# djene-mengistu/UAPS

Hardware: NVIDIA B200
Metric: fused_pl_kl_loss_pixels_per_s (higher is better)
Workload: dtype f32

## Files before the change

uaps_b200/csrc/common.cuh:

```cuda
#pragma once
#include <cuda_runtime.h>
#include <stdint.h>
#include <cstdlib>
#include "uaps_b200.h"

#define UAPS_API extern "C" __attribute__((visibility("default")))

#define UAPS_LAUNCH_CHECK()                                   \
    do {                                                      \
        cudaError_t e__ = cudaGetLastError();                 \
        if (e__ != cudaSuccess) return (int)e__;              \
    } while (0)

namespace uaps {

constexpr int kWarp = 32;

struct DeviceInfo { int sm_count; int cc_major; int cc_minor; };
inline const DeviceInfo& device_info() {
    static const DeviceInfo info = [] {
        DeviceInfo d{148, 10, 0};
        int dev = 0;
        if (cudaGetDevice(&dev) == cudaSuccess) {
            cudaDeviceGetAttribute(&d.sm_count, cudaDevAttrMultiProcessorCount, dev);
            cudaDeviceGetAttribute(&d.cc_major, cudaDevAttrComputeCapabilityMajor, dev);
            cudaDeviceGetAttribute(&d.cc_minor, cudaDevAttrComputeCapabilityMinor, dev);
        }
        return d;
    }();
    return info;
}

template <typename T> __host__ __device__ constexpr T ceil_div(T a, T b) { return (a + b - 1) / b; }

__device__ __forceinline__ void grid_dep_wait() { asm volatile("griddepcontrol.wait;" ::: "memory"); }
__device__ __forceinline__ void grid_dep_launch() { asm volatile("griddepcontrol.launch_dependents;" ::: "memory"); }
inline bool pdl_all_enabled() {
    static const bool on = [] { const char* e = getenv("UAPS_PDL"); return e != nullptr && atoi(e) != 0; }();
    return on;
}
template <typename... KArgs, typename... Args>
inline cudaError_t launch_k(void (*kern)(KArgs...), dim3 grid, dim3 block, size_t smem, cudaStream_t st, bool cooperative,
                            Args... args) {
    cudaLaunchConfig_t cfg{};
    cfg.gridDim = grid; cfg.blockDim = block; cfg.dynamicSmemBytes = smem; cfg.stream = st;
    cudaLaunchAttribute attr[2];
    int n = 0;
    if (pdl_all_enabled()) {
        attr[n].id = cudaLaunchAttributeProgrammaticStreamSerialization;
        attr[n].val.programmaticStreamSerializationAllowed = 1;
        ++n;
    }
    if (cooperative) {
        attr[n].id = cudaLaunchAttributeCooperative;
        attr[n].val.cooperative = 1;
        ++n;
    }
    cfg.attrs = attr; cfg.numAttrs = n;
    return cudaLaunchKernelEx(&cfg, kern, KArgs(args)...);
}
#define UAPS_LAUNCH(kern, grid, block, smem, stream, ...)                                          \
    do {                                                                                           \
        cudaError_t le__ = ::uaps::launch_k(kern, grid, block, smem, stream, false, __VA_ARGS__);  \
        if (le__ != cudaSuccess) return (int)le__;                                                 \
    } while (0)

inline bool aligned_to(const void* p, size_t a) { return (reinterpret_cast<uintptr_t>(p) % a) == 0; }

template <int VEC> struct VecF;
template <> struct VecF<4> { using type = float4; };
template <> struct VecF<2> { using type = float2; };
template <> struct VecF<1> { using type = float;  };

template <int VEC>
__device__ __forceinline__ void load_vec(const float* __restrict__ p, float (&out)[VEC]) {
    using V = typename VecF<VEC>::type;
    V v = __ldg(reinterpret_cast<const V*>(p));
    const float* f = reinterpret_cast<const float*>(&v);
#pragma unroll
    for (int i = 0; i < VEC; ++i) out[i] = f[i];
}
template <int VEC>
__device__ __forceinline__ void store_vec(float* __restrict__ p, const float (&in)[VEC]) {
    using V = typename VecF<VEC>::type;
    V v;
    float* f = reinterpret_cast<float*>(&v);
#pragma unroll
    for (int i = 0; i < VEC; ++i) f[i] = in[i];
    *reinterpret_cast<V*>(p) = v;
}

__device__ __forceinline__ float warp_sum(float v) {
#pragma unroll
    for (int o = 16; o > 0; o >>= 1) v += __shfl_xor_sync(0xffffffffu, v, o);
    return v;
}
__device__ __forceinline__ double warp_sum(double v) {
#pragma unroll
    for (int o = 16; o > 0; o >>= 1) v += __shfl_xor_sync(0xffffffffu, v, o);
    return v;
}
__device__ __forceinline__ float warp_max(float v) {
#pragma unroll
    for (int o = 16; o > 0; o >>= 1) v = fmaxf(v, __shfl_xor_sync(0xffffffffu, v, o));
    return v;
}

__host__ __device__ __forceinline__ uint32_t enc_ordered(float f) {
#ifdef __CUDA_ARCH__
// ... 35 lines not shown
```

uaps_b200/csrc/fused_loss.cu:

```cuda
#define UAPS_LOSS_ENTRY
#include <cstdlib>
#include <cstring>
#include "fused_loss_impl.cuh"

namespace uaps {
namespace loss {
#define UAPS_DECL_K(KK)                                                                                       \
    extern template int launch_loss_k<KK>(int, int, bool, bool, const LossArgs&, float*, const float*,       \
                                          const float*, int*, cudaStream_t);
UAPS_DECL_K(1) UAPS_DECL_K(2) UAPS_DECL_K(3) UAPS_DECL_K(4) UAPS_DECL_K(5) UAPS_DECL_K(6)
#undef UAPS_DECL_K
}

namespace {
using namespace loss;

int check_common(const float* const* z, int K, int B, int C, int64_t HW, const float* mix_w,
                 const int64_t* labels, const float* wcw_dev) {
    if (z == nullptr || B <= 0 || HW <= 0) return UAPS_EINVAL;
    if (K < 1 || K > KMAX || C < 2 || C > CMAX) return UAPS_ERANGE;
    if (labels == nullptr && mix_w == nullptr && wcw_dev == nullptr) return UAPS_EINVAL;
    if ((double)B * (double)HW >= 2147483648.0) return UAPS_ERANGE;
    for (int k = 0; k < K; ++k) {
        if (z[k] == nullptr) return UAPS_EINVAL;
        if (!aligned_to(z[k], 4)) return UAPS_EALIGN;
    }
    if (labels != nullptr && !aligned_to(labels, 8)) return UAPS_EALIGN;
    return UAPS_OK;
}

int pick_vec(const float* const* z, float* const* o, int K, int64_t HW) {
    int vec = (HW % 4 == 0) ? 4 : (HW % 2 == 0 ? 2 : 1);
    for (int k = 0; k < K; ++k) {
        while (vec > 1 && !aligned_to(z[k], 4 * vec)) vec >>= 1;
        if (o != nullptr && o[k] != nullptr)
            while (vec > 1 && !aligned_to(o[k], 4 * vec)) vec >>= 1;
    }
    return vec;
}


int pick_impl(int avail_vec, int flags, bool pass2, int kc) {
    static const int forced = [] { const char* e = getenv("UAPS_LOSS_IMPL"); return e ? atoi(e) : -1; }();
    static const int forced_p1 = [] { const char* e = getenv("UAPS_LOSS_P1_IMPL"); return e ? atoi(e) : -1; }();
    if (flags & UAPS_LOSS_EXACT) return IMPL_EXACT;
    if (avail_vec < 2) return IMPL_SCALAR;
    if (!pass2 && forced_p1 >= 0 && forced_p1 != IMPL_EXACT && forced_p1 <= IMPL_VEC4 && (forced_p1 != IMPL_VEC4 || avail_vec >= 4) &&
        (forced_p1 != IMPL_VEC4_PF || avail_vec >= 4))
        return forced_p1;
    if (forced >= 0 && forced <= IMPL_SCALAR) return forced;
    if (avail_vec < 4) return IMPL_VEC2_PF;
    static const int p2_vec4_max_kc = [] { const char* e = getenv("UAPS_LOSS_P2_VEC4_MAXKC"); return e ? atoi(e) : 12; }();
    if (pass2) return kc <= p2_vec4_max_kc ? IMPL_VEC4_PF : IMPL_VEC2_PF;
    return IMPL_VEC4_PF;
}

int dispatch_k(int K, int C, int impl, bool sup, bool pass2, const LossArgs& a, float* partials, const float* sc,
               const float* go, int* nblocks, cudaStream_t st) {
    switch (K) {
        case 1: return launch_loss_k<1>(C, impl, sup, pass2, a, partials, sc, go, nblocks, st);
        case 2: return launch_loss_k<2>(C, impl, sup, pass2, a, partials, sc, go, nblocks, st);
        case 3: return launch_loss_k<3>(C, impl, sup, pass2, a, partials, sc, go, nblocks, st);
        case 4: return launch_loss_k<4>(C, impl, sup, pass2, a, partials, sc, go, nblocks, st);
        case 5: return launch_loss_k<5>(C, impl, sup, pass2, a, partials, sc, go, nblocks, st);
        case 6: return launch_loss_k<6>(C, impl, sup, pass2, a, partials, sc, go, nblocks, st);
    }
    return UAPS_ERANGE;
}


constexpr int XCHG_WMAX = UAPS_XCHG_MAX_RANKS;
constexpr int XCHG_SLOT = 128;
constexpr size_t XCHG_WORDS = (size_t)2 * XCHG_WMAX * 2 * XCHG_SLOT;
constexpr size_t XCHG_STATUS_OFF = XCHG_WORDS * sizeof(unsigned long long);
constexpr size_t XCHG_BYTES = XCHG_STATUS_OFF + 128;
static_assert(sums_count(KMAX, CMAX) <= XCHG_SLOT, "slot too small");

struct ExchangeArgs {
    char* box[XCHG_WMAX];
    int rank, world;
    unsigned epoch;
    const unsigned* epoch_dev;
    unsigned long long timeout_ns;
};

__device__ __forceinline__ void st_word_sys(unsigned long long* p, unsigned data, unsigned flag) {
    asm volatile("st.volatile.global.v2.u32 [%0], {%1, %2};" ::"l"(p), "r"(data), "r"(flag) : "memory");
}
__device__ __forceinline__ void ld_word_sys(const unsigned long long* p, unsigned& data, unsigned& flag) {
    asm volatile("ld.volatile.global.v2.u32 {%0, %1}, [%2];" : "=r"(data), "=r"(flag) : "l"(p) : "memory");
}
__device__ __forceinline__ unsigned long long global_timer_ns() {
    unsigned long long t;
    asm volatile("mov.u64 %0, %%globaltimer;" : "=l"(t));
    return t;
}

__global__ void __launch_bounds__(1024) loss_fold_exchange_finalize_kernel(const float* __restrict__ partials, int S, unsigned nblocks,
                                                                            double* __restrict__ sums, const ExchangeArgs x, int K,
                                                                            int C, double N, float cw1, float cw2, int supervised,
                                                                            float* __restrict__ sc, int nsc,
                                                                            const float* __restrict__ wcw_dev) {
    __shared__ double s_sums[XCHG_SLOT];
    __shared__ double s_term[KMAX * CMAX];
    __shared__ int s_timed_out;
    pdl_trigger();
    pdl_wait();
    const unsigned epoch = x.epoch + (x.epoch_dev != nullptr ? *x.epoch_dev : 0u);
    if (wcw_dev != nullptr) { cw1 = wcw_dev[UAPS_WCW_CW1]; cw2 = wcw_dev[UAPS_WCW_CW2]; }
    if (threadIdx.x == 0) s_timed_out = 0;
    cta_fold_rows(partials, S, nblocks, s_sums);
    __shared__ unsigned s_words[XCHG_WMAX][2 * XCHG_SLOT];
    const int ph = epoch & 1;
    const int nw = 2 * S;
    for (int t = threadIdx.x; t < x.world * nw; t += blockDim.x) {
        const int p = t / nw, idx = t - p * nw;
        const unsigned bits = reinterpret_cast<const unsigned*>(s_sums)[idx];
        unsigned long long* dst = reinterpret_cast<unsigned long long*>(x.box[p]) +
                                  ((size_t)(ph * XCHG_WMAX + x.rank) * 2 * XCHG_SLOT + idx);
        st_word_sys(dst, bits, epoch);
    }
    int timed_out = 0;
    for (int t = threadIdx.x; t < x.world * nw; t += blockDim.x) {
        const int p = t / nw, idx = t - p * nw;
        const unsigned long long* src = reinterpret_cast<const unsigned long long*>(x.box[x.rank]) +
                                        ((size_t)(ph * XCHG_WMAX + p) * 2 * XCHG_SLOT + idx);
        unsigned data, flag;
        const unsigned long long t0 = global_timer_ns();
        for (;;) {
            ld_word_sys(src, data, flag);
            if (flag == epoch) break;
            if (*reinterpret_cast<volatile int*>(&s_timed_out) != 0 || global_timer_ns() - t0 > x.timeout_ns) {
                s_timed_out = 1; timed_out = 1; break;
            }
        }
        if (timed_out) break;
        s_words[p][idx] = data;
// ... 98 lines not shown
UAPS_API int uaps_xchg_alloc(void** mailbox) {
    if (mailbox == nullptr) return UAPS_EINVAL;
    cudaError_t e = cudaMalloc(mailbox, XCHG_BYTES);
    if (e != cudaSuccess) return (int)e;
    e = cudaMemset(*mailbox, 0, XCHG_BYTES);
    if (e == cudaSuccess) e = cudaDeviceSynchronize();
    return (int)e;
}
UAPS_API int uaps_xchg_free(void* mailbox) { return mailbox ? (int)cudaFree(mailbox) : UAPS_OK; }

UAPS_API int uaps_xchg_export(void* mailbox, void* handle64) {
    if (mailbox == nullptr || handle64 == nullptr) return UAPS_EINVAL;
    static_assert(sizeof(cudaIpcMemHandle_t) == 64, "handle size");
    return (int)cudaIpcGetMemHandle(reinterpret_cast<cudaIpcMemHandle_t*>(handle64), mailbox);
}
UAPS_API int uaps_xchg_import(const void* handle64, void** peer_mailbox) {
    if (handle64 == nullptr || peer_mailbox == nullptr) return UAPS_EINVAL;
    cudaIpcMemHandle_t h;
    memcpy(&h, handle64, sizeof(h));
    const cudaError_t e = cudaIpcOpenMemHandle(peer_mailbox, h, cudaIpcMemLazyEnablePeerAccess);
    if (e != cudaSuccess) (void)cudaGetLastError();
    return (int)e;
}
UAPS_API int uaps_xchg_close(void* peer_mailbox) { return peer_mailbox ? (int)cudaIpcCloseMemHandle(peer_mailbox) : UAPS_OK; }

UAPS_API int uaps_xchg_status(const void* mailbox, unsigned* status_out, cudaStream_t stream) {
    if (mailbox == nullptr || status_out == nullptr) return UAPS_EINVAL;
    cudaError_t e = cudaMemcpyAsync(status_out, reinterpret_cast<const char*>(mailbox) + XCHG_STATUS_OFF, sizeof(unsigned),
                                    cudaMemcpyDeviceToHost, stream);
    if (e == cudaSuccess) e = cudaStreamSynchronize(stream);
    return (int)e;
}

UAPS_API int uaps_loss_pass1_exchange(const float* const* z, int K, int B, int C, int64_t HW, const float* mix_w,
                                      const int64_t* labels, void* workspace, double* sums, int64_t* pseudo_out,
                                      float* const* exp_var_out, int flags, void* const* mailboxes, int rank, int world,
                                      unsigned epoch, int64_t N_global, float cw1, float cw2, float* scalars,
                                      const float* wcw_dev, const uint32_t* epoch_dev, cudaStream_t stream) {
    if (scalars == nullptr || mailboxes == nullptr || N_global <= 0 || epoch == 0) return UAPS_EINVAL;
    if ((wcw_dev != nullptr && !aligned_to(wcw_dev, 4)) || (epoch_dev != nullptr && !aligned_to(epoch_dev, 4))) return UAPS_EALIGN;
    if (world < 1 || world > XCHG_WMAX || rank < 0 || rank >= world) return UAPS_ERANGE;
    if (!aligned_to(scalars, 4)) return UAPS_EALIGN;
    ExchangeArgs x{};
    for (int p = 0; p < world; ++p) {
        if (mailboxes[p] == nullptr) return UAPS_EINVAL;
        if (!aligned_to(mailboxes[p], 128)) return UAPS_EALIGN;
        x.box[p] = reinterpret_cast<char*>(mailboxes[p]);
    }
    x.rank = rank; x.world = world; x.epoch = epoch; x.epoch_dev = epoch_dev;
    const char* tmo = getenv("UAPS_XCHG_TIMEOUT_MS");
    x.timeout_ns = (tmo ? strtoull(tmo, nullptr, 10) : 30000ull) * 1000000ull;
    return loss_pass1_impl(z, K, B, C, HW, mix_w, labels, workspace, sums, pseudo_out, exp_var_out, flags, stream, N_global, cw1,
                           cw2, scalars, &x, wcw_dev);
}


UAPS_API int uaps_loss_finalize(const double* sums_global, int K, int C, int64_t N_global, float cw1,
                                  float cw2, int supervised, float* scalars, cudaStream_t stream) {
    if (sums_global == nullptr || scalars == nullptr || N_global <= 0) return UAPS_EINVAL;
    if (K < 1 || K > KMAX || C < 2 || C > CMAX) return UAPS_ERANGE;
    if (!aligned_to(sums_global, 8) || !aligned_to(scalars, 4)) return UAPS_EALIGN;
    const int rc = (int)launch_pdl(loss_finalize_kernel, dim3(1), dim3(32), stream, pdl_enabled(), sums_global, K, C, (double)N_global,
                                   cw1, cw2, supervised, scalars);
    if (rc != 0) return rc;
    UAPS_LAUNCH_CHECK();
    return UAPS_OK;
}

UAPS_API int uaps_loss_pass2(const float* const* z, int K, int B, int C, int64_t HW, const float* mix_w,
                               const int64_t* labels, const float* scalars, const float* grad_out,
                               float* const* dz, int flags, const float* wcw_dev, cudaStream_t stream) {
    int rc = check_common(z, K, B, C, HW, mix_w, labels, wcw_dev);
    if (rc != UAPS_OK) return rc;
    if (scalars == nullptr || grad_out == nullptr || dz == nullptr) return UAPS_EINVAL;
    LossArgs a{};
    for (int k = 0; k < K; ++k) {
        if (dz[k] == nullptr) return UAPS_EINVAL;
        if (!aligned_to(dz[k], 4)) return UAPS_EALIGN;
        a.z[k] = z[k];
        a.w[k] = mix_w ? mix_w[k] : 0.f;
        a.out[k] = dz[k];
    }
    a.labels = labels; a.pseudo = nullptr; a.HW = HW; a.B = B; a.w_dev = labels == nullptr ? wcw_dev : nullptr;
    const int impl = pick_impl(pick_vec(z, dz, K, HW), flags, true, K * C);
    int nblocks = 0;
    return dispatch_k(K, C, impl, labels != nullptr, true, a, nullptr, scalars, grad_out, &nblocks, stream);
}
```

uaps_b200/csrc/fused_loss_impl.cuh:

```cuda
#pragma once
#include <cstdlib>
#include "common.cuh"

namespace uaps {
namespace loss {

constexpr int KMAX = UAPS_KMAX;
constexpr int CMAX = UAPS_CMAX;
constexpr int LOSS_THREADS = 128;
constexpr int LOSS_MAX_BLOCKS = 640;
constexpr int WS_HEADER_BYTES = 256;

__host__ __device__ constexpr int sums_count(int K, int C) { return 3 * K + 2 * K * C + C; }
__host__ __device__ constexpr int min_ctas(int K, int C, int VEC, bool pass1) {
#ifdef UAPS_P1_CTAS
    if (pass1) return UAPS_P1_CTAS;
#endif
    const int need = K * C * VEC + (pass1 ? sums_count(K, C) : K * C) + 64;
    return need <= 124 ? 4 : (need <= 176 ? 3 : 2);
}
__host__ __device__ constexpr int scalars_count(int K, int C) { return UAPS_SC_BASE + 4 * K + 2 * K * C; }

__device__ __forceinline__ void pdl_wait() { asm volatile("griddepcontrol.wait;" ::: "memory"); }
__device__ __forceinline__ void pdl_trigger() { asm volatile("griddepcontrol.launch_dependents;" ::: "memory"); }

template <typename... KArgs, typename... Args>
inline cudaError_t launch_pdl(void (*kern)(KArgs...), dim3 grid, dim3 block, cudaStream_t st, bool pdl, Args... args) {
    cudaLaunchConfig_t cfg{};
    cfg.gridDim = grid; cfg.blockDim = block; cfg.dynamicSmemBytes = 0; cfg.stream = st;
    cudaLaunchAttribute attr[1];
    attr[0].id = cudaLaunchAttributeProgrammaticStreamSerialization;
    attr[0].val.programmaticStreamSerializationAllowed = 1;
    cfg.attrs = attr; cfg.numAttrs = pdl ? 1 : 0;
    return cudaLaunchKernelEx(&cfg, kern, KArgs(args)...);
}
inline bool pdl_enabled() {
    static const bool on = [] { const char* e = getenv("UAPS_LOSS_PDL"); return e == nullptr || atoi(e) != 0; }();
    return on;
}

struct LossArgs {
    const float* z[KMAX];
    float* out[KMAX];
    float w[KMAX];
    const float* w_dev;
    const int64_t* labels;
    int64_t* pseudo;
    long long HW;
    unsigned groups_per_image;
    unsigned ngroups;
    int B;
    int write_ev;
};

template <bool EXACT> struct LogUnit { static constexpr float U = EXACT ? 1.0f : 0.6931471805599453f; };

template <int K, int C>
struct PixelState {
    float p[K][C];
    float l[K][C];
    float q[C];
    float lq[C];
    float V[K];
    float E[K];
    int y;
};

template <int C>
__device__ __forceinline__ void softmax_exact(const float (&z)[C], float (&p)[C], float (&l)[C]) {
    float m = z[0];
#pragma unroll
    for (int c = 1; c < C; ++c) m = fmaxf(m, z[c]);
    float e[C];
    float s = 0.f;
#pragma unroll
    for (int c = 0; c < C; ++c) {
        e[c] = expf(__fsub_rn(z[c], m));
        s = __fadd_rn(s, e[c]);
    }
    const float ls = logf(s);
#pragma unroll
    for (int c = 0; c < C; ++c) {
        p[c] = __fdiv_rn(e[c], s);
        l[c] = __fsub_rn(__fsub_rn(z[c], m), ls);
    }
}

__device__ __forceinline__ float ex2_approx(float x) { float y; asm("ex2.approx.ftz.f32 %0, %1;" : "=f"(y) : "f"(x)); return y; }
__device__ __forceinline__ float lg2_approx(float x) { float y; asm("lg2.approx.ftz.f32 %0, %1;" : "=f"(y) : "f"(x)); return y; }
__device__ __forceinline__ float rcp_approx(float x) { float y; asm("rcp.approx.ftz.f32 %0, %1;" : "=f"(y) : "f"(x)); return y; }
constexpr float kLog2e = 1.4426950408889634f;
constexpr float kTieMargin = 2e-5f;
constexpr float kLg2Floor = -120.0f;

template <int C, bool TRACK_MIN>
__device__ __forceinline__ float softmax_fast(const float (&z)[C], float (&p)[C], float (&l2)[C]) {
    float m = z[0];
#pragma unroll
    for (int c = 1; c < C; ++c) m = fmaxf(m, z[c]);
    const float nm = -m * kLog2e;
    float e[C];
    float s = 0.f, tmin = 0.f;
#pragma unroll
    for (int c = 0; c < C; ++c) {
        const float t = fmaf(z[c], kLog2e, nm);
        if constexpr (TRACK_MIN) tmin = fminf(tmin, t);
        e[c] = ex2_approx(t);
        s += e[c];
    }
    const float r = rcp_approx(s);
#pragma unroll
    for (int c = 0; c < C; ++c) {
        p[c] = e[c] * r;
        l2[c] = lg2_approx(p[c]);
    }
    return tmin;
}

template <int C>
__device__ __forceinline__ void log2_softmax_underflow_fix(const float (&z)[C], float (&l2)[C]) {
    float m = z[0];
#pragma unroll
    for (int c = 1; c < C; ++c) m = fmaxf(m, z[c]);
    float t[C], s = 0.f;
#pragma unroll
    for (int c = 0; c < C; ++c) { t[c] = (z[c] - m) * kLog2e; s += ex2_approx(t[c]); }
    const float l2s = lg2_approx(s);
#pragma unroll
    for (int c = 0; c < C; ++c)
        if (t[c] < kLg2Floor) l2[c] = t[c] - l2s;
}

template <int K>
// ... 144 lines not shown
    int y = 0;
    float best = st.q[0], second = -1.f;
#pragma unroll
    for (int c = 1; c < C; ++c) {
        if (st.q[c] > best) { second = best; best = st.q[c]; y = c; }
        else second = fmaxf(second, st.q[c]);
    }
    float vs = st.V[0];
#pragma unroll
    for (int k = 1; k < K; ++k) vs += st.V[k];
    const bool tie = !(best - second > kTieMargin);
    const bool bad = !(fabsf(vs) < 1e30f);
    if (__builtin_expect(tie || bad, 0)) {
        if (tie) y = argmax_exact_gmem<K, C, true>(a, pix_off);
        if (bad) {
#pragma unroll
            for (int k = 0; k < K; ++k) log2_softmax_underflow_fix<C>(z[k], st.l[k]);
            kl_terms<K, C, false, true>(st);
        }
    }
    st.y = y;
}

template <int K, int C, int VEC, typename Args>
__device__ __forceinline__ void load_group(const Args& a, unsigned g, float (&zv)[K][C][VEC]) {
    const unsigned b = g / a.groups_per_image;
    const unsigned hw = (g - b * a.groups_per_image) * VEC;
    const size_t base = (size_t)b * C * a.HW + hw;
#pragma unroll
    for (int k = 0; k < K; ++k)
#pragma unroll
        for (int c = 0; c < C; ++c) load_vec<VEC>(a.z[k] + base + (size_t)c * a.HW, zv[k][c]);
}

template <int K, int C>
struct AccIdx {
    static constexpr int CE = 0, E = K, V = 2 * K, I = 3 * K, P = 3 * K + K * C, T = 3 * K + 2 * K * C;
    static constexpr int S = 3 * K + 2 * K * C + C;
};

template <int K, int C, bool EXACT>
__device__ __forceinline__ void accumulate_pixel(const PixelState<K, C>& st, float (&acc)[AccIdx<K, C>::S]) {
    using AI = AccIdx<K, C>;
    constexpr float U = LogUnit<EXACT>::U;
    float oh[C];
#pragma unroll
    for (int c = 0; c < C; ++c) {
        oh[c] = (st.y == c) ? 1.f : 0.f;
        acc[AI::T + c] += oh[c];
    }
#pragma unroll
    for (int k = 0; k < K; ++k) {
        acc[AI::E + k] += st.E[k];
        acc[AI::V + k] += st.V[k];
        float ly = 0.f;
#pragma unroll
        for (int c = 0; c < C; ++c) {
            ly = fmaf(oh[c], st.l[k][c], ly);
            acc[AI::I + k * C + c] = fmaf(oh[c], st.p[k][c], acc[AI::I + k * C + c]);
            acc[AI::P + k * C + c] += st.p[k][c];
        }
        acc[AI::CE + k] = fmaf(-U, ly, acc[AI::CE + k]);
    }
}

template <int S, int THREADS>
__device__ __forceinline__ void block_store_partials(float (&acc)[S], float* __restrict__ partials,
                                                     float (*s_red)[S]) {
    const int lane = threadIdx.x & 31, warp = threadIdx.x >> 5;
#pragma unroll
    for (int i = 0; i < S; ++i) {
        const float r = warp_sum(acc[i]);
        if (lane == 0) s_red[warp][i] = r;
    }
    __syncthreads();
    for (int i = threadIdx.x; i < S; i += THREADS) {
        float r = 0.f;
#pragma unroll
        for (int wv = 0; wv < THREADS / kWarp; ++wv) r += s_red[wv][i];
        partials[(size_t)i * LOSS_MAX_BLOCKS + blockIdx.x] = r;
    }
}

template <int K, int C, int VEC, bool SUP, bool EXACT, bool PF, bool WDEV>
__global__ void __launch_bounds__(LOSS_THREADS, min_ctas(K, C, PF ? 2 * VEC : VEC, true))
loss_pass1_kernel(const __grid_constant__ LossArgs a, float* __restrict__ partials) {
    constexpr int S = sums_count(K, C);
    __shared__ float s_red[LOSS_THREADS / kWarp][S];
    pdl_wait();
    pdl_trigger();

    float w[K];
#pragma unroll
    for (int k = 0; k < K; ++k) w[k] = WDEV ? a.w_dev[k] : a.w[k];

    float acc[S];
#pragma unroll
    for (int i = 0; i < S; ++i) acc[i] = 0.f;

    const unsigned stride = gridDim.x * LOSS_THREADS;
    unsigned g = blockIdx.x * LOSS_THREADS + threadIdx.x;
    float zn[PF ? K : 1][PF ? C : 1][PF ? VEC : 1];
    if constexpr (PF) { if (g < a.ngroups) load_group<K, C, VEC>(a, g, zn); }
    for (; g < a.ngroups; g += stride) {
        const unsigned b = g / a.groups_per_image;
        const unsigned hw = (g - b * a.groups_per_image) * VEC;
        const size_t base = (size_t)b * C * a.HW + hw;
        float zv[K][C][VEC];
        if constexpr (PF) {
#pragma unroll
            for (int k = 0; k < K; ++k)
#pragma unroll
                for (int c = 0; c < C; ++c)
#pragma unroll
                    for (int j = 0; j < VEC; ++j) zv[k][c][j] = zn[k][c][j];
            if (g + stride < a.ngroups) load_group<K, C, VEC>(a, g + stride, zn);
        } else {
            load_group<K, C, VEC>(a, g, zv);
        }
        long long lab[VEC];
        if constexpr (SUP) {
#pragma unroll
            for (int j = 0; j < VEC; ++j) lab[j] = __ldg(a.labels + (size_t)b * a.HW + hw + j);
        }
        float ev[K][VEC];
        long long yv[VEC];
#pragma unroll
        for (int j = 0; j < VEC; ++j) {
            float z[K][C];
#pragma unroll
            for (int k = 0; k < K; ++k)
#pragma unroll
                for (int c = 0; c < C; ++c) z[k][c] = zv[k][c][j];
            PixelState<K, C> st;
            pixel_forward<K, C, SUP, EXACT>(z, w, SUP ? (int)lab[j] : 0, a, base + j, st);
            yv[j] = st.y;
#pragma unroll
            for (int k = 0; k < K; ++k) ev[k][j] = st.E[k];
            accumulate_pixel<K, C, EXACT>(st, acc);
        }
        if (a.pseudo != nullptr) {
#pragma unroll
            for (int j = 0; j < VEC; ++j) a.pseudo[(size_t)b * a.HW + hw + j] = yv[j];
        }
        if (a.write_ev) {
#pragma unroll
            for (int k = 0; k < K; ++k)
                if (a.out[k] != nullptr) store_vec<VEC>(a.out[k] + (size_t)b * a.HW + hw, ev[k]);
        }
    }

    block_store_partials<S, LOSS_THREADS>(acc, partials, s_red);
}

#ifdef UAPS_LOSS_ENTRY
__global__ void __launch_bounds__(256) loss_fold_kernel(const float* __restrict__ partials, int S, unsigned nblocks,
                                                        double* __restrict__ sums) {
    pdl_trigger();
    pdl_wait();
    const int lane = threadIdx.x & 31;
    const int i = blockIdx.x * (256 / kWarp) + (threadIdx.x >> 5);
    if (i >= S) return;
    const float* row = partials + (size_t)i * LOSS_MAX_BLOCKS;
    float v[LOSS_MAX_BLOCKS / kWarp];
#pragma unroll
    for (int u = 0; u < LOSS_MAX_BLOCKS / kWarp; ++u) {
        const unsigned blk = u * kWarp + lane;
        v[u] = (blk < nblocks) ? __ldcg(row + blk) : 0.f;
    }
    double r = 0.0;
#pragma unroll
    for (int u = 0; u < LOSS_MAX_BLOCKS / kWarp; ++u) r += (double)v[u];
    r = warp_sum(r);
    if (lane == 0) sums[i] = r;
}

__device__ __forceinline__ void cta_fold_rows(const float* __restrict__ partials, int S, unsigned nblocks, double* s_sums) {
    constexpr int HALF = 16, PER_LANE = LOSS_MAX_BLOCKS / HALF;
    const int sub = threadIdx.x & (HALF - 1);
    for (int base = (threadIdx.x >> 5) * 2; base < S; base += 2 * (1024 / 32)) {
        const int i = base + ((threadIdx.x >> 4) & 1);
        const bool live = i < S;
        const float* row = partials + (size_t)(live ? i : 0) * LOSS_MAX_BLOCKS;
        float v[PER_LANE];
#pragma unroll
        for (int u = 0; u < PER_LANE; ++u) {
            const unsigned blk = u * HALF + sub;
            v[u] = (live && blk < nblocks) ? __ldcg(row + blk) : 0.f;
        }
        double r = 0.0;
#pragma unroll
        for (int u = 0; u < PER_LANE; ++u) r += (double)v[u];
#pragma unroll
        for (int o = HALF / 2; o > 0; o >>= 1) r += __shfl_xor_sync(0xffffffffu, r, o);
        if (live && sub == 0) s_sums[i] = r;
    }
    __syncthreads();
}

__device__ __forceinline__ void cta_finalize(const double* sums, int K, int C, double N, float cw1, float cw2, int supervised,
                                             float* sc, double* s_term) {
    const double* sI = sums + 3 * K;
    const double* sP = sums + 3 * K + K * C;
    const double* sT = sums + 3 * K + 2 * K * C;
    float* Ikc = sc + UAPS_SC_BASE + 4 * K;
    float* Card = Ikc + K * C;
    const int t = threadIdx.x;
    if (t < K * C) {
        const double card = sP[t] + sT[t % C];
        s_term[t] = 2.0 * sI[t] / (card + 1e-7);
        Ikc[t] = (float)sI[t];
        Card[t] = (float)card;
    }
    __syncthreads();
    if (t != 0) return;
    const double* sCE = sums;
    const double* sE = sums + K;
    const double* sV = sums + 2 * K;
    float* ps = sc + UAPS_SC_BASE;
    float* Eb = ps + K;
    float* CE = Eb + K;
    float* DI = CE + K;
    const double invN = 1.0 / N;
    double ps_loss = 0.0, unc = 0.0, mce = 0.0, mdi = 0.0;
    for (int k = 0; k < K; ++k) {
        const double ce = sCE[k] / N;
        double d = 0.0;
        for (int c = 0; c < C; ++c) d += s_term[k * C + c];
        const double dice = 1.0 - d / C;
        const double psk = 0.5 * (ce + dice);
        const double eb = supervised ? 1.0 : sE[k] / N;
// ... 77 lines not shown
__global__ void loss_finalize_kernel(const double* __restrict__ sums, int K, int C, double N,
                                     float cw1, float cw2, int supervised, float* __restrict__ sc) {
    pdl_trigger();
    pdl_wait();
    if (threadIdx.x != 0 || blockIdx.x != 0) return;
    finalize_from_sums(sums, K, C, N, cw1, cw2, supervised, sc);
}
#endif

template <int K, int C>
struct GradConsts {
    float psk[K];
    float cce[K];
    float A[K][C];
    float Bc[K][C];
    float lam1, lam2, invNK;
};

template <int K, int C>
__device__ __forceinline__ void load_grad_consts(GradConsts<K, C>& gc, const float* __restrict__ sc,
                                                 const float* __restrict__ grad_out) {
    const float g_loss = grad_out[UAPS_SC_LOSS_U], g_ps = grad_out[UAPS_SC_PS_LOSS], g_unc = grad_out[UAPS_SC_L_UNCERT];
    const float g_ce = grad_out[UAPS_SC_MEAN_CE], g_dice = grad_out[UAPS_SC_MEAN_DICE];
    const float lam1 = g_loss * sc[UAPS_SC_CW1] + g_ps;
    const float lam2 = g_loss * sc[UAPS_SC_CW2] + g_unc;
    const float invN = sc[UAPS_SC_INV_N];
    const float* ps = sc + UAPS_SC_BASE;
    const float* Eb = ps + K;
    const float* Ikc = ps + 4 * K;
    const float* Card = Ikc + K * C;
    gc.lam1 = lam1; gc.lam2 = lam2; gc.invNK = invN / K;
    for (int k = 0; k < K; ++k) {
        gc.psk[k] = ps[k];
        const float half = lam1 * Eb[k] / (2.f * K);
        const float dce = half + g_ce / K;
        const float ddice = half + g_dice / K;
        gc.cce[k] = dce * invN;
        for (int c = 0; c < C; ++c) {
            const float den = Card[k * C + c] + 1e-7f;
            gc.A[k][c] = -ddice * (2.f / C) / den;
            gc.Bc[k][c] = ddice * (2.f / C) * Ikc[k * C + c] / (den * den);
        }
    }
}

template <int K, int C, bool SUP, bool EXACT>
__device__ __forceinline__ void pixel_backward(const PixelState<K, C>& st, const GradConsts<K, C>& gc,
                                               float (&dz)[K][C]) {
    float gk[K];
    float Gq[C];
#pragma unroll
    for (int c = 0; c < C; ++c) Gq[c] = 0.f;
    if constexpr (!SUP) {
#pragma unroll
        for (int k = 0; k < K; ++k) {
            gk[k] = (gc.lam2 - gc.lam1 * gc.psk[k] * st.E[k]) * gc.invNK;
#pragma unroll
            for (int c = 0; c < C; ++c) Gq[c] += gk[k] * fmaf(LogUnit<EXACT>::U, st.lq[c] - st.l[k][c], 1.f);
        }
#pragma unroll
        for (int c = 0; c < C; ++c) Gq[c] *= (1.0f / K);
    }
    float oh[C];
#pragma unroll
    for (int c = 0; c < C; ++c) oh[c] = (st.y == c) ? 1.f : 0.f;
#pragma unroll
    for (int k = 0; k < K; ++k) {
        float Gl[C], Gp[C];
        float sGl = 0.f, dot = 0.f;
#pragma unroll
        for (int c = 0; c < C; ++c) {
            float gl = -gc.cce[k] * oh[c];
            if constexpr (!SUP) gl = fmaf(-gk[k], st.q[c], gl);
            const float gp = fmaf(gc.A[k][c], oh[c], Gq[c] + gc.Bc[k][c]);
            Gl[c] = gl; Gp[c] = gp;
            sGl += gl;
            dot = fmaf(st.p[k][c], gp, dot);
        }
#pragma unroll
        for (int c = 0; c < C; ++c) dz[k][c] = fmaf(st.p[k][c], (Gp[c] - dot) - sGl, Gl[c]);
    }
}

template <int K, int C, int VEC, bool SUP, bool EXACT, bool PF, bool WDEV>
__global__ void __launch_bounds__(LOSS_THREADS, min_ctas(K, C, PF ? 2 * VEC : VEC, false))
loss_pass2_kernel(const __grid_constant__ LossArgs a, const float* __restrict__ sc, const float* __restrict__ grad_out) {
    __shared__ GradConsts<K, C> gc;

    float w[K];
#pragma unroll
    for (int k = 0; k < K; ++k) w[k] = WDEV ? a.w_dev[k] : a.w[k];

    const unsigned stride = gridDim.x * LOSS_THREADS;
    unsigned g = blockIdx.x * LOSS_THREADS + threadIdx.x;
    float zn[PF ? K : 1][PF ? C : 1][PF ? VEC : 1];
    if constexpr (PF) { if (g < a.ngroups) load_group<K, C, VEC>(a, g, zn); }
    pdl_wait();
    pdl_trigger();
    if (threadIdx.x == 0) load_grad_consts<K, C>(gc, sc, grad_out);
    __syncthreads();
    for (; g < a.ngroups; g += stride) {
        const unsigned b = g / a.groups_per_image;
        const unsigned hw = (g - b * a.groups_per_image) * VEC;
        const size_t base = (size_t)b * C * a.HW + hw;
        float zv[K][C][VEC];
        if constexpr (PF) {
#pragma unroll
            for (int k = 0; k < K; ++k)
#pragma unroll
                for (int c = 0; c < C; ++c)
#pragma unroll
                    for (int j = 0; j < VEC; ++j) zv[k][c][j] = zn[k][c][j];
            if (g + stride < a.ngroups) load_group<K, C, VEC>(a, g + stride, zn);
        } else {
            load_group<K, C, VEC>(a, g, zv);
        }
        long long lab[VEC];
        if constexpr (SUP) {
#pragma unroll
            for (int j = 0; j < VEC; ++j) lab[j] = __ldg(a.labels + (size_t)b * a.HW + hw + j);
        }
#pragma unroll
        for (int j = 0; j < VEC; ++j) {
            float z[K][C];
#pragma unroll
            for (int k = 0; k < K; ++k)
#pragma unroll
                for (int c = 0; c < C; ++c) z[k][c] = zv[k][c][j];
            PixelState<K, C> st;
            pixel_forward<K, C, SUP, EXACT>(z, w, SUP ? (int)lab[j] : 0, a, base + j, st);
            float dz[K][C];
            pixel_backward<K, C, SUP, EXACT>(st, gc, dz);
#pragma unroll
            for (int k = 0; k < K; ++k)
#pragma unroll
                for (int c = 0; c < C; ++c) zv[k][c][j] = dz[k][c];
        }
#pragma unroll
        for (int k = 0; k < K; ++k)
#pragma unroll
            for (int c = 0; c < C; ++c) store_vec<VEC>(a.out[k] + base + (size_t)c * a.HW, zv[k][c]);
    }
}

enum LossImpl { IMPL_VEC4_PF = 0, IMPL_VEC2_PF = 1, IMPL_SCALAR = 2, IMPL_EXACT = 3, IMPL_VEC2 = 4, IMPL_VEC4 = 5 };

__host__ __device__ constexpr bool has_vec4(int K, int C) { return K * C <= 16; }
__host__ __device__ constexpr bool has_vec2(int K, int C) { return K * C <= 24; }

template <typename Kern>
inline int grid_for(Kern kern, unsigned ngroups) {
    int occ = 1;
    if (cudaOccupancyMaxActiveBlocksPerMultiprocessor(&occ, kern, LOSS_THREADS, 0) != cudaSuccess || occ < 1) occ = 1;
    long long want = ceil_div<long long>(ngroups, LOSS_THREADS);
    long long cap = (long long)device_info().sm_count * occ;
    if (cap > LOSS_MAX_BLOCKS) cap = LOSS_MAX_BLOCKS;
    return (int)(want < cap ? want : cap);
}

template <int K, int C, int VEC, bool SUP, bool EXACT, bool PF, bool WDEV>
inline int launch_reg(bool pass2, LossArgs a, float* partials, const float* sc, const float* go, int* nblocks,
                      cudaStream_t st) {
    a.groups_per_image = (unsigned)(a.HW / VEC);
    a.ngroups = (unsigned)a.B * a.groups_per_image;
    if (!pass2) {
        auto kern = loss_pass1_kernel<K, C, VEC, SUP, EXACT, PF, WDEV>;
        static const int grid_cap = grid_for(kern, 0x7fffffffu);
        const long long want = ceil_div<long long>(a.ngroups, LOSS_THREADS);
        *nblocks = (int)(want < grid_cap ? want : grid_cap);
        const cudaError_t e = launch_pdl(kern, dim3(*nblocks), dim3(LOSS_THREADS), st, pdl_enabled(), a, partials);
        if (e != cudaSuccess) return (int)e;
    } else {
        auto kern = loss_pass2_kernel<K, C, VEC, SUP, EXACT, PF, WDEV>;
        static const int grid_cap = grid_for(kern, 0x7fffffffu);
        const long long want = ceil_div<long long>(a.ngroups, LOSS_THREADS);
        *nblocks = (int)(want < grid_cap ? want : grid_cap);
        const cudaError_t e = launch_pdl(kern, dim3(*nblocks), dim3(LOSS_THREADS), st, pdl_enabled(), a, sc, go);
        if (e != cudaSuccess) return (int)e;
    }
    UAPS_LAUNCH_CHECK();
    return UAPS_OK;
}

template <int K, int C>
inline int launch_kc(int impl, bool sup, bool pass2, const LossArgs& a, float* partials, const float* sc,
                     const float* go, int* nblocks, cudaStream_t st) {
#define UAPS_RUN(VEC, EXACT, PF)                                                                       \
    (sup ? launch_reg<K, C, VEC, true, EXACT, PF, false>(pass2, a, partials, sc, go, nblocks, st)                      \
         : (a.w_dev != nullptr ? launch_reg<K, C, VEC, false, EXACT, PF, true>(pass2, a, partials, sc, go, nblocks, st) \
                               : launch_reg<K, C, VEC, false, EXACT, PF, false>(pass2, a, partials, sc, go, nblocks, st)))
    if (impl == IMPL_EXACT) return UAPS_RUN(1, true, false);
#ifdef UAPS_LOSS_EXTRA_VARIANTS
    if constexpr (has_vec2(K, C)) { if (impl == IMPL_VEC2) return UAPS_RUN(2, false, false); }
    if constexpr (has_vec4(K, C)) { if (impl == IMPL_VEC4) return UAPS_RUN(4, false, false); }
#endif
    if constexpr (has_vec4(K, C)) { if (impl == IMPL_VEC4_PF) return UAPS_RUN(4, false, true); }
    if constexpr (has_vec2(K, C)) { if (impl == IMPL_VEC4_PF || impl == IMPL_VEC2_PF) return UAPS_RUN(2, false, true); }
    return UAPS_RUN(1, false, false);
#undef UAPS_RUN
}

template <int K>
int launch_loss_k(int C, int impl, bool sup, bool pass2, const LossArgs& a, float* partials, const float* sc,
                  const float* go, int* nblocks, cudaStream_t st) {
    switch (C) {
        case 2: return launch_kc<K, 2>(impl, sup, pass2, a, partials, sc, go, nblocks, st);
        case 3: return launch_kc<K, 3>(impl, sup, pass2, a, partials, sc, go, nblocks, st);
        case 4: return launch_kc<K, 4>(impl, sup, pass2, a, partials, sc, go, nblocks, st);
        case 5: return launch_kc<K, 5>(impl, sup, pass2, a, partials, sc, go, nblocks, st);
        case 6: return launch_kc<K, 6>(impl, sup, pass2, a, partials, sc, go, nblocks, st);
        case 7: return launch_kc<K, 7>(impl, sup, pass2, a, partials, sc, go, nblocks, st);
        case 8: return launch_kc<K, 8>(impl, sup, pass2, a, partials, sc, go, nblocks, st);
    }
    return UAPS_ERANGE;
}

}
}
```

Measured before the change: 23.93 billion.

## Stage pass-1 inputs via cp.async ring and rotate pass-2 to hit L2-resident tail

Pass 1 now prefetches the next pixel group into a double-buffered shared-memory ring with cp.async instead of register prefetch. Each thread processes one pixel per group from shared memory and parks its outputs in the consumed slot before storing them. Pass 2 starts its traversal at the tail of the tensor, whose size is derived from the L2 capacity, so it reuses data pass 1 left in L2. It also marks its loads and stores evict-first. This adds dynamic shared memory, which can lower occupancy, and changes the launch-bounds hints.

Result: slower. 22.96 billion (median of 6 runs) (-4.1%).

```diff
diff --git a/uaps_b200/csrc/common.cuh b/uaps_b200/csrc/common.cuh
--- a/uaps_b200/csrc/common.cuh
+++ b/uaps_b200/csrc/common.cuh
@@ -16,15 +16,16 @@
 
 constexpr int kWarp = 32;
 
-struct DeviceInfo { int sm_count; int cc_major; int cc_minor; };
+struct DeviceInfo { int sm_count; int cc_major; int cc_minor; int l2_bytes; };
 inline const DeviceInfo& device_info() {
     static const DeviceInfo info = [] {
-        DeviceInfo d{148, 10, 0};
+        DeviceInfo d{148, 10, 0, 0};
         int dev = 0;
         if (cudaGetDevice(&dev) == cudaSuccess) {
             cudaDeviceGetAttribute(&d.sm_count, cudaDevAttrMultiProcessorCount, dev);
             cudaDeviceGetAttribute(&d.cc_major, cudaDevAttrComputeCapabilityMajor, dev);
             cudaDeviceGetAttribute(&d.cc_minor, cudaDevAttrComputeCapabilityMinor, dev);
+            cudaDeviceGetAttribute(&d.l2_bytes, cudaDevAttrL2CacheSize, dev);
         }
         return d;
     }();
diff --git a/uaps_b200/csrc/fused_loss.cu b/uaps_b200/csrc/fused_loss.cu
--- a/uaps_b200/csrc/fused_loss.cu
+++ b/uaps_b200/csrc/fused_loss.cu
@@ -53,6 +53,12 @@
     static const int p2_vec4_max_kc = [] { const char* e = getenv("UAPS_LOSS_P2_VEC4_MAXKC"); return e ? atoi(e) : 12; }();
     if (pass2) return kc <= p2_vec4_max_kc ? IMPL_VEC4_PF : IMPL_VEC2_PF;
     return IMPL_VEC4_PF;
+}
+
+constexpr double kL2TailFraction = 0.5;
+unsigned pass2_first_pixel(int K, int C, long long npix) {
+    const long long tail = (long long)(kL2TailFraction * device_info().l2_bytes / (sizeof(float) * K * C));
+    return tail > 0 && npix > tail ? (unsigned)(npix - tail) : 0u;
 }
 
 int dispatch_k(int K, int C, int impl, bool sup, bool pass2, const LossArgs& a, float* partials, const float* sc,
@@ -317,6 +323,7 @@
         a.out[k] = dz[k];
     }
     a.labels = labels; a.pseudo = nullptr; a.HW = HW; a.B = B; a.w_dev = labels == nullptr ? wcw_dev : nullptr;
+    a.first_pixel = pass2_first_pixel(K, C, (long long)B * HW);
     const int impl = pick_impl(pick_vec(z, dz, K, HW), flags, true, K * C);
     int nblocks = 0;
     return dispatch_k(K, C, impl, labels != nullptr, true, a, nullptr, scalars, grad_out, &nblocks, stream);
diff --git a/uaps_b200/csrc/fused_loss_impl.cuh b/uaps_b200/csrc/fused_loss_impl.cuh
--- a/uaps_b200/csrc/fused_loss_impl.cuh
+++ b/uaps_b200/csrc/fused_loss_impl.cuh
@@ -25,14 +25,19 @@
 __device__ __forceinline__ void pdl_trigger() { asm volatile("griddepcontrol.launch_dependents;" ::: "memory"); }
 
 template <typename... KArgs, typename... Args>
-inline cudaError_t launch_pdl(void (*kern)(KArgs...), dim3 grid, dim3 block, cudaStream_t st, bool pdl, Args... args) {
+inline cudaError_t launch_pdl_smem(void (*kern)(KArgs...), dim3 grid, dim3 block, size_t smem, cudaStream_t st, bool pdl,
+                                   Args... args) {
     cudaLaunchConfig_t cfg{};
-    cfg.gridDim = grid; cfg.blockDim = block; cfg.dynamicSmemBytes = 0; cfg.stream = st;
+    cfg.gridDim = grid; cfg.blockDim = block; cfg.dynamicSmemBytes = smem; cfg.stream = st;
     cudaLaunchAttribute attr[1];
     attr[0].id = cudaLaunchAttributeProgrammaticStreamSerialization;
     attr[0].val.programmaticStreamSerializationAllowed = 1;
     cfg.attrs = attr; cfg.numAttrs = pdl ? 1 : 0;
     return cudaLaunchKernelEx(&cfg, kern, KArgs(args)...);
+}
+template <typename... KArgs, typename... Args>
+inline cudaError_t launch_pdl(void (*kern)(KArgs...), dim3 grid, dim3 block, cudaStream_t st, bool pdl, Args... args) {
+    return launch_pdl_smem(kern, grid, block, 0, st, pdl, args...);
 }
 inline bool pdl_enabled() {
     static const bool on = [] { const char* e = getenv("UAPS_LOSS_PDL"); return e == nullptr || atoi(e) != 0; }();
@@ -49,6 +54,8 @@
     long long HW;
     unsigned groups_per_image;
     unsigned ngroups;
+    unsigned first_pixel;
+    unsigned g0;
     int B;
     int write_ev;
 };
@@ -359,71 +366,131 @@
     }
 }
 
+template <int K, int C, int VEC>
+__host__ __device__ constexpr size_t stage_floats() { return (size_t)K * C * LOSS_THREADS * VEC; }
+template <int K, int C, int VEC>
+__host__ __device__ constexpr size_t ring_bytes() { return 2 * stage_floats<K, C, VEC>() * sizeof(float); }
+
+template <int VEC>
+__device__ __forceinline__ void cp_async_vec(float* smem, const float* gmem) {
+    const unsigned s = (unsigned)__cvta_generic_to_shared(smem);
+    if constexpr (VEC == 4) asm volatile("cp.async.cg.shared.global [%0], [%1], 16;" ::"r"(s), "l"(gmem) : "memory");
+    else asm volatile("cp.async.ca.shared.global [%0], [%1], 8;" ::"r"(s), "l"(gmem) : "memory");
+}
+__device__ __forceinline__ void cp_async_commit() { asm volatile("cp.async.commit_group;" ::: "memory"); }
+__device__ __forceinline__ void cp_async_wait_prev() { asm volatile("cp.async.wait_group 1;" ::: "memory"); }
+
+template <int K, int C, int VEC>
+__device__ __forceinline__ void stage_group(const LossArgs& a, unsigned g, float* slot) {
+    const unsigned b = g / a.groups_per_image;
+    const unsigned hw = (g - b * a.groups_per_image) * VEC;
+    const size_t base = (size_t)b * C * a.HW + hw;
+#pragma unroll
+    for (int k = 0; k < K; ++k)
+#pragma unroll
+        for (int c = 0; c < C; ++c) cp_async_vec<VEC>(slot + (k * C + c) * LOSS_THREADS * VEC, a.z[k] + base + (size_t)c * a.HW);
+}
+
 template <int K, int C, int VEC, bool SUP, bool EXACT, bool PF, bool WDEV>
-__global__ void __launch_bounds__(LOSS_THREADS, min_ctas(K, C, PF ? 2 * VEC : VEC, true))
+__global__ void __launch_bounds__(LOSS_THREADS, min_ctas(K, C, PF ? 2 : VEC, true))
 loss_pass1_kernel(const __grid_constant__ LossArgs a, float* __restrict__ partials) {
     constexpr int S = sums_count(K, C);
+    constexpr int PIX = PF ? 1 : VEC;
     __shared__ float s_red[LOSS_THREADS / kWarp][S];
+    extern __shared__ __align__(16) float s_ring[];
     pdl_wait();
     pdl_trigger();
 
-    float w[K];
-#pragma unroll
-    for (int k = 0; k < K; ++k) w[k] = WDEV ? a.w_dev[k] : a.w[k];
-
     float acc[S];
 #pragma unroll
     for (int i = 0; i < S; ++i) acc[i] = 0.f;
 
     const unsigned stride = gridDim.x * LOSS_THREADS;
     unsigned g = blockIdx.x * LOSS_THREADS + threadIdx.x;
-    float zn[PF ? K : 1][PF ? C : 1][PF ? VEC : 1];
-    if constexpr (PF) { if (g < a.ngroups) load_group<K, C, VEC>(a, g, zn); }
-    for (; g < a.ngroups; g += stride) {
+    float* const slot0 = s_ring + threadIdx.x * VEC;
+    constexpr size_t SF = stage_floats<K, C, VEC>();
+    if constexpr (PF) {
+        if (g < a.ngroups) stage_group<K, C, VEC>(a, g, slot0);
+        cp_async_commit();
+    }
+    for (unsigned it = 0; g < a.ngroups; g += stride, ++it) {
         const unsigned b = g / a.groups_per_image;
         const unsigned hw = (g - b * a.groups_per_image) * VEC;
         const size_t base = (size_t)b * C * a.HW + hw;
-        float zv[K][C][VEC];
+        float zv[PF ? 1 : K][PF ? 1 : C][PF ? 1 : VEC];
+        const float* cur = slot0 + (it & 1) * SF;
         if constexpr (PF) {
-#pragma unroll
-            for (int k = 0; k < K; ++k)
-#pragma unroll
-                for (int c = 0; c < C; ++c)
-#pragma unroll
-                    for (int j = 0; j < VEC; ++j) zv[k][c][j] = zn[k][c][j];
-            if (g + stride < a.ngroups) load_group<K, C, VEC>(a, g + stride, zn);
+            if (g + stride < a.ngroups) stage_group<K, C, VEC>(a, g + stride, slot0 + ((it & 1) ^ 1) * SF);
+            cp_async_commit();
+            cp_async_wait_prev();
         } else {
             load_group<K, C, VEC>(a, g, zv);
         }
-        long long lab[VEC];
-        if constexpr (SUP) {
-#pragma unroll
-            for (int j = 0; j < VEC; ++j) lab[j] = __ldg(a.labels + (size_t)b * a.HW + hw + j);
-        }
-        float ev[K][VEC];
-        long long yv[VEC];
-#pragma unroll
-        for (int j = 0; j < VEC; ++j) {
-            float z[K][C];
+        float ev[PF ? 1 : K][PF ? 1 : VEC];
+        long long yv[PF ? 1 : VEC];
+        float* const park = const_cast<float*>(cur);
+#pragma unroll 1
+        for (int j0 = 0; j0 < VEC; j0 += PIX) {
+            const int jpf = PF ? (j0 + (int)(threadIdx.x / (kWarp / VEC))) & (VEC - 1) : j0;
+            float zp[K][C][PIX];
 #pragma unroll
             for (int k = 0; k < K; ++k)
 #pragma unroll
-                for (int c = 0; c < C; ++c) z[k][c] = zv[k][c][j];
-            PixelState<K, C> st;
-            pixel_forward<K, C, SUP, EXACT>(z, w, SUP ? (int)lab[j] : 0, a, base + j, st);
-            yv[j] = st.y;
-#pragma unroll
-            for (int k = 0; k < K; ++k) ev[k][j] = st.E[k];
-            accumulate_pixel<K, C, EXACT>(st, acc);
-        }
-        if (a.pseudo != nullptr) {
-#pragma unroll
-            for (int j = 0; j < VEC; ++j) a.pseudo[(size_t)b * a.HW + hw + j] = yv[j];
-        }
-        if (a.write_ev) {
-#pragma unroll
-            for (int k = 0; k < K; ++k)
-                if (a.out[k] != nullptr) store_vec<VEC>(a.out[k] + (size_t)b * a.HW + hw, ev[k]);
+                for (int c = 0; c < C; ++c) {
+                    if constexpr (PF) {
+                        zp[k][c][0] = cur[(k * C + c) * LOSS_THREADS * VEC + jpf];
+                    } else {
+#pragma unroll
+                        for (int j = 0; j < PIX; ++j) zp[k][c][j] = zv[k][c][j0 + j];
+                    }
+                }
+#pragma unroll
+            for (int jj = 0; jj < PIX; ++jj) {
+                const int j = jpf + jj;
+                float z[K][C];
+#pragma unroll
+                for (int k = 0; k < K; ++k)
+#pragma unroll
+                    for (int c = 0; c < C; ++c) z[k][c] = zp[k][c][jj];
+                float w[K];
+#pragma unroll
+                for (int k = 0; k < K; ++k) w[k] = WDEV ? __ldg(a.w_dev + k) : a.w[k];
+                PixelState<K, C> st;
+                const int label = SUP ? (int)__ldg(a.labels + (size_t)b * a.HW + hw + j) : 0;
+                pixel_forward<K, C, SUP, EXACT>(z, w, label, a, base + j, st);
+                if constexpr (PF) {
+                    park[K * LOSS_THREADS * VEC + j] = __int_as_float(st.y);
+#pragma unroll
+                    for (int k = 0; k < K; ++k) park[k * LOSS_THREADS * VEC + j] = st.E[k];
+                } else {
+                    yv[j] = st.y;
+#pragma unroll
+                    for (int k = 0; k < K; ++k) ev[k][j] = st.E[k];
+                }
+                accumulate_pixel<K, C, EXACT>(st, acc);
+            }
+        }
+        if constexpr (PF) {
+            static_assert(!PF || K + 1 <= K * C, "the parked outputs need K + 1 planes");
+            if (a.pseudo != nullptr) {
+#pragma unroll
+                for (int j = 0; j < VEC; ++j) a.pseudo[(size_t)b * a.HW + hw + j] = __float_as_int(park[K * LOSS_THREADS * VEC + j]);
+            }
+            if (a.write_ev) {
+#pragma unroll
+                for (int k = 0; k < K; ++k)
+                    if (a.out[k] != nullptr) store_vec<VEC>(a.out[k] + (size_t)b * a.HW + hw, *reinterpret_cast<const float (*)[VEC]>(park + k * LOSS_THREADS * VEC));
+            }
+        } else {
+            if (a.pseudo != nullptr) {
+#pragma unroll
+                for (int j = 0; j < VEC; ++j) a.pseudo[(size_t)b * a.HW + hw + j] = yv[j];
+            }
+            if (a.write_ev) {
+#pragma unroll
+                for (int k = 0; k < K; ++k)
+                    if (a.out[k] != nullptr) store_vec<VEC>(a.out[k] + (size_t)b * a.HW + hw, ev[k]);
+            }
         }
     }
 
@@ -667,6 +734,46 @@
     }
 }
 
+__device__ __forceinline__ unsigned long long l2_evict_first_policy() {
+    unsigned long long p;
+    asm volatile("createpolicy.fractional.L2::evict_first.b64 %0, 1.0;" : "=l"(p));
+    return p;
+}
+template <int VEC>
+__device__ __forceinline__ void load_vec_hint(const float* p, float (&o)[VEC], unsigned long long pol) {
+    if constexpr (VEC == 4)
+        asm("ld.global.nc.L2::cache_hint.v4.f32 {%0, %1, %2, %3}, [%4], %5;"
+            : "=f"(o[0]), "=f"(o[1]), "=f"(o[2]), "=f"(o[3]) : "l"(p), "l"(pol));
+    else if constexpr (VEC == 2)
+        asm("ld.global.nc.L2::cache_hint.v2.f32 {%0, %1}, [%2], %3;" : "=f"(o[0]), "=f"(o[1]) : "l"(p), "l"(pol));
+    else
+        asm("ld.global.nc.L2::cache_hint.f32 %0, [%1], %2;" : "=f"(o[0]) : "l"(p), "l"(pol));
+}
+template <int VEC>
+__device__ __forceinline__ void store_vec_hint(float* p, const float (&v)[VEC], unsigned long long pol) {
+    if constexpr (VEC == 4)
+        asm volatile("st.global.L2::cache_hint.v4.f32 [%0], {%1, %2, %3, %4}, %5;"
+                     ::"l"(p), "f"(v[0]), "f"(v[1]), "f"(v[2]), "f"(v[3]), "l"(pol) : "memory");
+    else if constexpr (VEC == 2)
+        asm volatile("st.global.L2::cache_hint.v2.f32 [%0], {%1, %2}, %3;" ::"l"(p), "f"(v[0]), "f"(v[1]), "l"(pol) : "memory");
+    else
+        asm volatile("st.global.L2::cache_hint.f32 [%0], %1, %2;" ::"l"(p), "f"(v[0]), "l"(pol) : "memory");
+}
+template <int K, int C, int VEC>
+__device__ __forceinline__ void load_group_hint(const LossArgs& a, unsigned g, float (&zv)[K][C][VEC], unsigned long long pol) {
+    const unsigned b = g / a.groups_per_image;
+    const unsigned hw = (g - b * a.groups_per_image) * VEC;
+    const size_t base = (size_t)b * C * a.HW + hw;
+#pragma unroll
+    for (int k = 0; k < K; ++k)
+#pragma unroll
+        for (int c = 0; c < C; ++c) load_vec_hint<VEC>(a.z[k] + base + (size_t)c * a.HW, zv[k][c], pol);
+}
+__device__ __forceinline__ unsigned rotate_group(const LossArgs& a, unsigned g) {
+    const unsigned r = g + a.g0;
+    return r >= a.ngroups ? r - a.ngroups : r;
+}
+
 template <int K, int C, int VEC, bool SUP, bool EXACT, bool PF, bool WDEV>
 __global__ void __launch_bounds__(LOSS_THREADS, min_ctas(K, C, PF ? 2 * VEC : VEC, false))
 loss_pass2_kernel(const __grid_constant__ LossArgs a, const float* __restrict__ sc, const float* __restrict__ grad_out) {
@@ -676,17 +783,19 @@
 #pragma unroll
     for (int k = 0; k < K; ++k) w[k] = WDEV ? a.w_dev[k] : a.w[k];
 
+    const unsigned long long pol = l2_evict_first_policy();
     const unsigned stride = gridDim.x * LOSS_THREADS;
     unsigned g = blockIdx.x * LOSS_THREADS + threadIdx.x;
     float zn[PF ? K : 1][PF ? C : 1][PF ? VEC : 1];
-    if constexpr (PF) { if (g < a.ngroups) load_group<K, C, VEC>(a, g, zn); }
+    if constexpr (PF) { if (g < a.ngroups) load_group_hint<K, C, VEC>(a, rotate_group(a, g), zn, pol); }
     pdl_wait();
     pdl_trigger();
     if (threadIdx.x == 0) load_grad_consts<K, C>(gc, sc, grad_out);
     __syncthreads();
     for (; g < a.ngroups; g += stride) {
-        const unsigned b = g / a.groups_per_image;
-        const unsigned hw = (g - b * a.groups_per_image) * VEC;
+        const unsigned gr = rotate_group(a, g);
+        const unsigned b = gr / a.groups_per_image;
+        const unsigned hw = (gr - b * a.groups_per_image) * VEC;
         const size_t base = (size_t)b * C * a.HW + hw;
         float zv[K][C][VEC];
         if constexpr (PF) {
@@ -696,9 +805,9 @@
                 for (int c = 0; c < C; ++c)
 #pragma unroll
                     for (int j = 0; j < VEC; ++j) zv[k][c][j] = zn[k][c][j];
-            if (g + stride < a.ngroups) load_group<K, C, VEC>(a, g + stride, zn);
+            if (g + stride < a.ngroups) load_group_hint<K, C, VEC>(a, rotate_group(a, g + stride), zn, pol);
         } else {
-            load_group<K, C, VEC>(a, g, zv);
+            load_group_hint<K, C, VEC>(a, gr, zv, pol);
         }
         long long lab[VEC];
         if constexpr (SUP) {
@@ -724,7 +833,7 @@
 #pragma unroll
         for (int k = 0; k < K; ++k)
 #pragma unroll
-            for (int c = 0; c < C; ++c) store_vec<VEC>(a.out[k] + base + (size_t)c * a.HW, zv[k][c]);
+            for (int c = 0; c < C; ++c) store_vec_hint<VEC>(a.out[k] + base + (size_t)c * a.HW, zv[k][c], pol);
     }
 }
 
@@ -734,9 +843,9 @@
 __host__ __device__ constexpr bool has_vec2(int K, int C) { return K * C <= 24; }
 
 template <typename Kern>
-inline int grid_for(Kern kern, unsigned ngroups) {
+inline int grid_for(Kern kern, unsigned ngroups, size_t smem = 0) {
     int occ = 1;
-    if (cudaOccupancyMaxActiveBlocksPerMultiprocessor(&occ, kern, LOSS_THREADS, 0) != cudaSuccess || occ < 1) occ = 1;
+    if (cudaOccupancyMaxActiveBlocksPerMultiprocessor(&occ, kern, LOSS_THREADS, smem) != cudaSuccess || occ < 1) occ = 1;
     long long want = ceil_div<long long>(ngroups, LOSS_THREADS);
     long long cap = (long long)device_info().sm_count * occ;
     if (cap > LOSS_MAX_BLOCKS) cap = LOSS_MAX_BLOCKS;
@@ -750,12 +859,17 @@
     a.ngroups = (unsigned)a.B * a.groups_per_image;
     if (!pass2) {
         auto kern = loss_pass1_kernel<K, C, VEC, SUP, EXACT, PF, WDEV>;
-        static const int grid_cap = grid_for(kern, 0x7fffffffu);
+        constexpr size_t smem = PF ? ring_bytes<K, C, VEC>() : 0;
+        static const int grid_cap = [&] {
+            if (smem > 0) (void)cudaFuncSetAttribute(kern, cudaFuncAttributeMaxDynamicSharedMemorySize, (int)smem);
+            return grid_for(kern, 0x7fffffffu, smem);
+        }();
         const long long want = ceil_div<long long>(a.ngroups, LOSS_THREADS);
         *nblocks = (int)(want < grid_cap ? want : grid_cap);
-        const cudaError_t e = launch_pdl(kern, dim3(*nblocks), dim3(LOSS_THREADS), st, pdl_enabled(), a, partials);
+        const cudaError_t e = launch_pdl_smem(kern, dim3(*nblocks), dim3(LOSS_THREADS), smem, st, pdl_enabled(), a, partials);
         if (e != cudaSuccess) return (int)e;
     } else {
+        a.g0 = a.first_pixel / VEC;
         auto kern = loss_pass2_kernel<K, C, VEC, SUP, EXACT, PF, WDEV>;
         static const int grid_cap = grid_for(kern, 0x7fffffffu);
         const long long want = ceil_div<long long>(a.ngroups, LOSS_THREADS);
```
